# kupc25648/MOP-truss-MARL

Measured on AMD Instinct MI355X. Metric: env steps/sec (batched FEM solves) at 4096 envs, higher is better.
Workload: dtype f64; 1 GPU; synthetic random-geometry 2-row trusses, 32 nodes / 80 elements / 60 DOF, FEM-only env.step (action decode + FP64 assembly/solve + stresses + point), no agent; envs_per_gpu=4096, global_envs=4096, nodes=32, elements=80, ndof=60, half_bandwidth=7, lanes_per_env=16, rows_per_lane=1, parallelism=env-batch sharded over 1 GPU(s), no data-path collective

## Files before the change

mop-truss-marl_amd/csrc/truss_body.h:

```cpp
#pragma once
#include <stdint.h>
#include <math.h>

#ifndef TB_SCHED_FENCE
#define TB_SCHED_FENCE()
#endif
#ifndef TRUSS_HD
#error "define TRUSS_HD (e.g. __device__ __forceinline__) before including truss_body.h"
#endif

#define TF_TOP 1
#define TF_RESX 2
#define TF_RESY 4
#define TF_LOAD_BRIDGE 8
#define TF_LOAD_ROOF 16

#define TB_NO_DECODE 0x1u
#define TB_CLAMP_INPLACE 0x2u
#define TB_EMIT_OBS 0x4u

#if defined(__clang__)
typedef uint32_t tb_u4 __attribute__((ext_vector_type(4)));
typedef uint32_t tb_u2 __attribute__((ext_vector_type(2)));
typedef float tb_f4 __attribute__((ext_vector_type(4)));
// ... 512 lines not shown
      S[a] = m;
      S[b] = m;
    }
  }

  TRUSS_HD double load_at(const TopoDev &T, int r) const {
    if (r < 0 || r >= T.ndof) return 0.0;
    int nd = t_posnode(T)[r];
    if (nd < 0) return 0.0;
    int fl = t_nflags(T)[nd >> 1] & (is_roof ? TF_LOAD_ROOF : TF_LOAD_BRIDGE);
    if (!fl) return 0.0;
    return (nd & 1) ? load_y : load_x;
  }
  TRUSS_HD int orig_pos(const TopoDev &T, int tm, int p) const { return tm ? T.ndof - 1 - p : p; }
  TRUSS_HD double team_load(const TopoDev &T, int tm, int p) const {
    if (T.nteams == 1) return load_at(T, p);
    if (tm == 0) return p < T.ndof - T.KA ? load_at(T, p) : 0.0;
    return p < T.KA ? load_at(T, T.ndof - 1 - p) : 0.0;
  }

  static constexpr bool EBATCH = RPL == 1 && W <= 8 && EPL <= 5;
  static constexpr int ECH = EBATCH ? EPL : 1;
  TRUSS_HD void phase_elements(const TopoDev &T, const StepArgsDev &A) {
    const float *Y = ysh(T), *X = xsh(T);
    const int32_t *S = secsh(T);
    const int16_t *CN = t_conn(T);
    const double *AR = t_area(T), *ISR = t_isr(T);
    double *K = kb(T);
    const int16_t *AC = t_asm(T);
    double *EV = evsh(T);
    if (g == 0) EV[3 * T.E] = EV[3 * T.E + 1] = EV[3 * T.E + 2] = 0.0;
#pragma unroll
    for (int c0 = 0; c0 < EPL; c0 += ECH) {
      int n0[ECH], n1[ECH], sc[ECH], ev[ECH];
      tb_u2 code[ECH];
      float x0[ECH], x1[ECH], y0[ECH], y1[ECH];
      double Aa[ECH];
#pragma unroll
      for (int j = 0; j < ECH; ++j) {
        const int i = c0 + j < EPL ? c0 + j : EPL - 1;
        const int e = g + G * i;
        const int ee = e < T.E ? e : T.E - 1;
        const uint32_t c = *(const uint32_t *)(CN + 2 * ee);
        n0[j] = (int)(int16_t)(c & 0xffffu);
        n1[j] = (int)(int16_t)(c >> 16);
        sc[j] = S[ee];
        code[j] = *(const tb_u2 *)(AC + 4 * ee);
        ev[j] = 3 * ee;
      }
#pragma unroll
      for (int j = 0; j < ECH; ++j) {
        x0[j] = X[n0[j]];
        x1[j] = X[n1[j]];
        y0[j] = Y[n0[j]];
        y1[j] = Y[n1[j]];
        Aa[j] = AR[sc[j]];
      }
#pragma unroll
      for (int j = 0; j < ECH; ++j) {
        const int i = c0 + j;
        if (i < EPL) {
          const double dx = (double)x1[j] - (double)x0[j];
          const double dy = (double)y1[j] - (double)y0[j];
          const double l2 = dx * dx + dy * dy;
          const double rl = tb_rsqrt(l2);
          const double len = l2 * rl;
          const double c = dx * rl, s = dy * rl;
          const double k = (T.e_mod * Aa[j]) * rl;
          ek[i] = k;
          ec[i] = c;
          es[i] = s;
          ei[i] = ISR[sc[j]];
          if constexpr (EMIT) el[i] = (float)len;
          const double vol = (double)(float)(Aa[j] * len);
          if constexpr (EBATCH) p_vol += (g + G * i < T.E) ? vol : 0.0;
          else if (g + G * i < T.E) p_vol += vol;
          const double kc = k * c, ks = k * s;
          const double kcc = kc * c, kcs = kc * s, kss = ks * s;
          EV[ev[j] + 0] = kcc;
          EV[ev[j] + 1] = kcs;
          EV[ev[j] + 2] = kss;
          K[(int16_t)(code[j][0] & 0xffffu)] = -kcc;
          K[(int16_t)(code[j][0] >> 16)] = -kss;
          K[(int16_t)(code[j][1] & 0xffffu)] = -kcs;
          K[(int16_t)(code[j][1] >> 16)] = -kcs;
        }
      }
    }
  }

  TRUSS_HD void phase_assemble_nodes(const TopoDev &T) {
    const double *EV = evsh(T);
    const int16_t *AD = t_adj8(T), *DO = t_diagoff(T);
    double *K = kb(T);
    static_assert(NDEG == 8, "adjacency rows are read as one 16-byte unit");
    tb_u4 adj[NPL];
    int dof[NPL][3];
    double cc[NPL], cs[NPL], ss[NPL];
#pragma unroll
    for (int i = 0; i < NPL; ++i) {
      const int n0 = g + G * i, n = n0 < T.N ? n0 : T.N - 1;
      adj[i] = *(const tb_u4 *)(AD + n * NDEG);
      dof[i][0] = DO[3 * n];
      dof[i][1] = DO[3 * n + 1];
      dof[i][2] = DO[3 * n + 2];
      cc[i] = cs[i] = ss[i] = 0.0;
    }
#pragma unroll
    for (int h = 0; h < 2; ++h) {
      double ev[NPL][4][3];
#pragma unroll
      for (int i = 0; i < NPL; ++i)
#pragma unroll
        for (int a = 0; a < 4; ++a) {
          const uint32_t w = adj[i][2 * h + (a >> 1)];
          const int e = (a & 1) ? (int)(w >> 16) : (int)(w & 0xffffu);
          ev[i][a][0] = EV[3 * e + 0];
          ev[i][a][1] = EV[3 * e + 1];
          ev[i][a][2] = EV[3 * e + 2];
        }
#pragma unroll
      for (int i = 0; i < NPL; ++i)
#pragma unroll
        for (int a = 0; a < 4; ++a) {
          cc[i] += ev[i][a][0];
          cs[i] += ev[i][a][1];
          ss[i] += ev[i][a][2];
        }
    }
#pragma unroll
    for (int i = 0; i < NPL; ++i) {
      K[dof[i][0]] = cc[i];
      K[dof[i][1]] = ss[i];
      K[dof[i][2]] = cs[i];
    }
    for (int n = g + G * NPL; n < T.N; n += G) {
      double c2 = 0.0, s2 = 0.0, x2 = 0.0;
#pragma unroll
      for (int a = 0; a < NDEG; ++a) {
        const int e = AD[n * NDEG + a];
        c2 += EV[3 * e + 0];
        x2 += EV[3 * e + 1];
        s2 += EV[3 * e + 2];
      }
      K[DO[3 * n]] = c2;
      K[DO[3 * n + 1]] = s2;
      K[DO[3 * n + 2]] = x2;
    }
    const int idA = T.nteams == 1 ? T.ndof : T.ndof - T.KA;
    for (int r = idA + g; r < T.rowsA; r += G) K[r * W + r % W] = 1.0;
    for (int r = T.KA + T.mid + g; r < T.rowsB; r += G) K[(T.rowsA + r) * W + r % W] = 1.0;
  }

  TRUSS_HD void solver_scratch_init(const TopoDev &T) {
    double *Z = zs(T);
    const uint8_t *ZC = t_zcode(T);
    const int lbit = is_roof ? 4 : 2;
    {
      const int zt = T.zlen * T.nteams;
      constexpr int ZIT = 6;
#pragma unroll
      for (int i = 0; i < ZIT; ++i) {
        const int r0 = g + G * i, r = r0 < zt ? r0 : zt - 1;
        const int c = ZC[r];
        Z[r] = (c & lbit) ? ((c & 1) ? load_y : load_x) : 0.0;
      }
      for (int r = g + G * ZIT; r < zt; r += G) {
        const int c = ZC[r];
        Z[r] = (c & lbit) ? ((c & 1) ? load_y : load_x) : 0.0;
      }
    }
    tb_d2 *X2 = (tb_d2 *)__builtin_assume_aligned(xsol(T), 16);
    const tb_d2 z2 = {0.0, 0.0};
    for (int r = g; r < (T.zslot + 2) / 2; r += G) X2[r] = z2;
    double *RB = rbuf(T);
    for (int i = g; i < T.n_rest; i += G) RB[i] = 0.0;
  }

  TRUSS_HD void solver_init(const TopoDev &T) {
#pragma unroll
    for (int s = 0; s < RPL; ++s) {
      int r = gs + WL * s;
#pragma unroll
      for (int c = 0; c < W; ++c) R[s][c] = (c <= r) ? Kt[r * W + c] : Kt[c * W + r];
      rhs[s] = Zt[r];
    }
#pragma unroll
    for (int j = 0; j < W; ++j) xs[j] = 0.0;
  }

  double zkeep[RPL];
  TRUSS_HD void pivot_write(const TopoDev &T, int k, int kk) {
#pragma unroll
    for (int s = 0; s < RPL; ++s) Kt[k * W + gs + WL * s] = R[s][kk];
    bx = rhs[kk / WL];
  }
  TRUSS_HD void factor_z_store(const TopoDev &T, int kb, int c, int cnt) {
#pragma unroll
    for (int s = 0; s < RPL; ++s) {
      const int off = (gs + WL * s - c + W) % W;
      double *zp = off < cnt ? Zt + kb + off : ZRt + gs;
      *zp = zkeep[s];
    }
  }

  TRUSS_HD void pivot_update(const TopoDev &T, int k, int kk) {
    double col[W];
    {
      const double *Kn = Kt + (k + W) * W;
#pragma unroll
      for (int s = 0; s < RPL; ++s) ecol[s] = Kn[gs + WL * s];
    }
#pragma unroll
    for (int i = 0; i < W / 2; ++i) {
      tb_d2 v = ((const tb_d2 *)__builtin_assume_aligned(Kt + k * W, 16))[i];
      col[2 * i] = v[0];
      col[2 * i + 1] = v[1];
    }
    const double zk = tb_team_bcast(*this, kk % WL);
    if (gs == kk % WL) zkeep[kk / WL] = bx;
    const double d = col[kk];
    const double inv = tb_rcp(d);
#pragma unroll
    for (int s = 0; s < RPL; ++s) {
      double l = R[s][kk] * inv;
#pragma unroll
      for (int j = 0; j < W; ++j)
        if (j != kk) R[s][j] = fma(-l, col[j], R[s][j]);
      rhs[s] = fma(-l, zk, rhs[s]);
    }
#pragma unroll
    for (int s = 0; s < RPL; ++s) R[s][kk] = ecol[s];
    if (gs == kk % WL) {
      const int sp = kk / WL;
#pragma unroll
      for (int j = 0; j < W; ++j)
        if (j != kk) R[sp][j] = fr[sp][j];
      rhs[sp] = frhs[sp];
    }
  }
  double fr[RPL][W], frhs[RPL], ecol[RPL];
  TRUSS_HD void factor_rows_fetch(const TopoDev &T, int kb) {
#pragma unroll
    for (int s = 0; s < RPL; ++s) {
      const int rn = kb + W + gs + WL * s;
      const tb_d2 *K2 = (const tb_d2 *)__builtin_assume_aligned(Kt + rn * W, 16);
#pragma unroll
      for (int i = 0; i < W / 2; ++i) {
        tb_d2 v = K2[i];
        fr[s][2 * i] = v[0];
        fr[s][2 * i + 1] = v[1];
      }
      frhs[s] = Zt[rn];
    }
  }

  TRUSS_HD void pivot_check(const TopoDev &T) {
    const int lim = (T.nteams == 2 && team == 1) ? T.KA : (T.nteams == 2 ? T.KA + W : T.KA);
    for (int k = gs; k < lim; k += WL) {
      const double d = Kt[k * W + k % W];
      if (!(d > 0.0) || !(d < 1.7e308)) bad = 1;
    }
  }

  TRUSS_HD int win_row(const TopoDev &T, int slot) const { return T.KA + ((slot - T.KA % W + W) % W); }
  TRUSS_HD void merge_post(const TopoDev &T) {
    if (team == 1) {
      double *M = (double *)(L + T.o_mrg);
#pragma unroll
      for (int j = 0; j < W; ++j) M[gs * W + j] = R[0][j];
      M[W * W + gs] = rhs[0];
    }
  }
  TRUSS_HD void merge_take(const TopoDev &T) {
    if (team == 0) {
      const double *M = (const double *)(L + T.o_mrg);
      const int lim = T.ndof - T.KA;
      const int p = win_row(T, gs);
      const int pb = T.ndof - 1 - p;
#pragma unroll
      for (int j = 0; j < W; ++j) {
        const int c = win_row(T, j);
        const int cb = T.ndof - 1 - c;
        const bool ok = p < lim && c < lim;
        const double add = M[ok ? (pb % W) * W + (cb % W) : 0];
        R[0][j] += ok ? add : 0.0;
      }
      const double az = M[W * W + (p < lim ? pb % W : 0)];
      rhs[0] += p < lim ? az : 0.0;
    }
  }

  double bc[RPL][W], bz[RPL], bd[RPL];
  double nc[RPL][W], nz[RPL], nd[RPL];
  double bx;
  double myx[RPL] = {};
  TRUSS_HD void backsub_rows_fetch(const TopoDev &T, int kb) {
#pragma unroll
    for (int s = 0; s < RPL; ++s) {
      const int p = kb + gs + WL * s;
      const int pc = p < 0 ? 0 : p;
      const tb_d2 *K2 = (const tb_d2 *)__builtin_assume_aligned(Kt + pc * W, 16);
#pragma unroll
      for (int i = 0; i < W / 2; ++i) {
        tb_d2 v = K2[i];
        nc[s][2 * i] = v[0];
        nc[s][2 * i + 1] = v[1];
      }
      nz[s] = Zt[pc];
      nd[s] = Kt[pc * W + pc % W];
    }
  }
  TRUSS_HD void backsub_rows_adopt() {
#pragma unroll
    for (int s = 0; s < RPL; ++s) {
#pragma unroll
      for (int j = 0; j < W; ++j) bc[s][j] = nc[s][j];
      bz[s] = nz[s];
      bd[s] = tb_rcp(nd[s]);
    }
  }
  TRUSS_HD void backsub_step(const TopoDev &T, int k, int kk) {
    const int s = kk / WL;
    double acc0 = bz[s], acc1 = 0.0;
#pragma unroll
    for (int m = W - 1; m >= 2; --m) {
      const int j = (kk + m) % W;
      if (m & 1) acc1 = fma(-bc[s][j], xs[j], acc1);
      else acc0 = fma(-bc[s][j], xs[j], acc0);
    }
    const int jn = (kk + 1) % W;
    double acc = fma(-bc[s][jn], xs[jn], acc0 + acc1);
    bx = acc * bd[s];
  }
  TRUSS_HD void backsub_share(int kk) {
    xs[kk] = tb_team_bcast(*this, kk % WL);
    if (gs == kk % WL) myx[kk / WL] = bx;
  }
  TRUSS_HD bool owns_row(const TopoDev &T, int p) const {
    if (T.nteams == 1) return true;
    return team == 0 ? p < T.ndof - T.KA : p < T.KA;
  }
  TRUSS_HD void backsub_flush(const TopoDev &T, int kb) {
    double *XS = xsol(T);
#pragma unroll
    for (int s = 0; s < RPL; ++s) {
      const int p = kb + gs + WL * s;
      XS[owns_row(T, p) ? orig_pos(T, team, p) : T.zslot + 1] = myx[s];
    }
  }
  TRUSS_HD void backsub_flush_mid(const TopoDev &T) {
    double *XS = xsol(T);
    const int p = win_row(T, gs);
    XS[(team == 0 && owns_row(T, p)) ? p : T.zslot + 1] = myx[0];
  }
  TRUSS_HD void backsub_reload(const TopoDev &T) {
    const double *XS = xsol(T);
#pragma unroll
    for (int j = 0; j < W; ++j) {
      const int o = orig_pos(T, team, win_row(T, j));
      xs[j] = XS[(o >= 0 && o < T.ndof) ? o : T.zslot];
    }
  }

  TRUSS_HD float *oq0(const TopoDev &T) { return (float *)(L + T.o_kb + T.so_q0); }
  TRUSS_HD float *osr(const TopoDev &T) { return (float *)(L + T.o_kb + T.so_sr); }
  TRUSS_HD float *odisp(const TopoDev &T) { return (float *)(L + T.o_kb + T.so_disp); }
  TRUSS_HD float *omu(const TopoDev &T) { return (float *)(L + T.o_kb + T.so_mu); }
  TRUSS_HD float *omd(const TopoDev &T) { return (float *)(L + T.o_kb + T.so_md); }
  TRUSS_HD uint8_t *ocomp(const TopoDev &T) { return (uint8_t *)(L + T.o_kb + T.so_comp); }

  TRUSS_HD void phase_post_elements(const TopoDev &T, const StepArgsDev &A) {
    const double *XS = xsol(T);
    const int16_t *EX = t_exs(T);
    float *Q = oq0(T), *SR = osr(T);
    uint8_t *CP = ocomp(T);
    tb_u2 ex[EPL];
    double qv[EPL];
    float srv[EPL];
#pragma unroll
    for (int i = 0; i < EPL; ++i) {
      const int e = g + G * i;
      const int ee = e < T.E ? e : T.E - 1;
      ex[i] = *(const tb_u2 *)(EX + 4 * ee);
    }
    double v[EPL][4];
#pragma unroll
    for (int i = 0; i < EPL; ++i) {
      v[i][0] = XS[ex[i][0] & 0xffffu];
      v[i][1] = XS[ex[i][0] >> 16];
      v[i][2] = XS[ex[i][1] & 0xffffu];
      v[i][3] = XS[ex[i][1] >> 16];
    }
#pragma unroll
    for (int i = 0; i < EPL; ++i) {
      const double c = ec[i], s = es[i], k = ek[i];
      const double u0 = c * v[i][0] + s * v[i][1];
      const double u2 = c * v[i][2] + s * v[i][3];
      const double q = k * u0 + (-k) * u2;
      qv[i] = q;
      srv[i] = (float)(fabs(q) * ei[i]);
      p_c1 = fmaxf(p_c1, fabsf(srv[i]));
    }
#pragma unroll
    for (int i = 0; i < EPL; ++i) {
      const int e = g + G * i;
      const int ee = e < T.E ? e : T.E - 1;
      Q[ee] = (float)qv[i];
      SR[ee] = srv[i];
      CP[ee] = qv[i] > 0.0 ? 1 : 0;
      if constexpr (EMIT) {
        const bool cmp = qv[i] > 0.0;
        const float val = fminf(srv[i], 1.0f) * (srv[i] > 1.0f ? 1.0f : 0.5f);
        const tb_f2 tc = {cmp ? 0.0f : val, cmp ? val : 0.0f};
        ((tb_f2 *)((float *)L + T.b_tc))[ee] = tc;
        pe_sr[i] = srv[i];
        pe_cmp = i == 0 ? (cmp ? 1u : 0u) : (pe_cmp | (cmp ? 1u << i : 0u));
      }
    }
    if constexpr (EMIT) {
      if (g == 0) {
        const tb_f2 z = {0.0f, 0.0f};
        ((tb_f2 *)((float *)L + T.b_tc))[T.E] = z;
      }
    }
    if (A.q064 && active) {
      const size_t be = (size_t)envc * T.E;
#pragma unroll
      for (int i = 0; i < EPL; ++i) {
        const int e = g + G * i;
        if (e < T.E) A.q064[be + e] = qv[i];
      }
    }
    if (A.react) {
      const int16_t *CN = t_conn(T), *RS = t_restslot(T);
#pragma unroll
      for (int i = 0; i < EPL; ++i) {
        const int e = g + G * i;
        if (e < T.E) {
          const int n0 = CN[2 * e], n1 = CN[2 * e + 1];
          const double q = qv[i], c = ec[i], s = es[i];
          const int s0 = RS[2 * n0], s1 = RS[2 * n0 + 1];
          const int s2 = RS[2 * n1], s3 = RS[2 * n1 + 1];
          if (s0 >= 0) tb_lds_add(&rbuf(T)[s0], q * c);
          if (s1 >= 0) tb_lds_add(&rbuf(T)[s1], q * s);
          if (s2 >= 0) tb_lds_add(&rbuf(T)[s2], q * (-c));
          if (s3 >= 0) tb_lds_add(&rbuf(T)[s3], q * (-s));
        }
      }
    }
  }

  TRUSS_HD void phase_post_nodes(const TopoDev &T, const StepArgsDev &A) {
    const double *XS = xsol(T);
    const float *Y = ysh(T), *TG = tgsh(T);
    const int16_t *DP = t_dofpos(T), *PR = t_pairs(T);
    const uint8_t *NF = t_nflags(T);
    const size_t bn = (size_t)envc * T.N;
    const int zslot = T.zslot;
    float *DS = odisp(T), *MU = omu(T), *MD = omd(T);
    int px[NPL], py[NPL], fl[NPL];
    float yv[NPL], tg[NPL];
    double dxv[NPL], dyv[NPL];
#pragma unroll
    for (int i = 0; i < NPL; ++i) {
      const int n0 = g + G * i, n = n0 < T.N ? n0 : T.N - 1;
      px[i] = DP[2 * n];
      py[i] = DP[2 * n + 1];
      fl[i] = NF[n];
      yv[i] = Y[n];
      tg[i] = TG[n];
    }
#pragma unroll
    for (int i = 0; i < NPL; ++i) {
      dxv[i] = XS[px[i] < 0 ? zslot : px[i]];
      dyv[i] = XS[py[i] < 0 ? zslot : py[i]];
    }
#pragma unroll
    for (int i = 0; i < NPL; ++i) {
      const int n0 = g + G * i, n = n0 < T.N ? n0 : T.N - 1;
      const bool real = n0 < T.N, top = fl[i] & TF_TOP;
      const double dt = (double)fabsf(tg[i] - yv[i]);
      const float dr = fabsf((float)(dyv[i] / max_def));
      p_dt += (real && top) ? dt : 0.0;
      p_c2 = top ? p_c2 : fmaxf(p_c2, dr);
      DS[2 * n + 0] = (float)dxv[i];
      DS[2 * n + 1] = (float)dyv[i];
    }
    if (A.disp64 && active) {
#pragma unroll
      for (int i = 0; i < NPL; ++i) {
        const int n = g + G * i;
        if (n < T.N) {
          A.disp64[(bn + n) * 2 + 0] = dxv[i];
          A.disp64[(bn + n) * 2 + 1] = dyv[i];
        }
      }
    }
    for (int n = g + G * NPL; n < T.N; n += G) {
      const int qx = DP[2 * n], qy = DP[2 * n + 1];
      const double dx = XS[qx < 0 ? zslot : qx], dy = XS[qy < 0 ? zslot : qy];
      const float y = Y[n];
      if (NF[n] & TF_TOP) p_dt += (double)fabsf(TG[n] - y);
      else p_c2 = fmaxf(p_c2, fabsf((float)(dy / max_def)));
      DS[2 * n + 0] = (float)dx;
      DS[2 * n + 1] = (float)dy;
      if (A.disp64 && active) {
        A.disp64[(bn + n) * 2 + 0] = dx;
        A.disp64[(bn + n) * 2 + 1] = dy;
      }
    }
    if (A.mu_out && T.has_pairs) {
      constexpr int PPL = (NPL + 1) / 2;
#pragma unroll
// ... 270 lines not shown
        const int nc = n < T.N ? n : T.N - 1;
        const int fl = NFL[nc];
        const float y = Y[nc];
        float *f = nfe[i];
        f[0] = X[nc];
        f[1] = y;
        f[2] = (fl & lbit) ? 1.0f : 0.0f;
        f[3] = MU[nc];
        f[4] = MD[nc];
        f[5] = (fl & TF_TOP) ? TG[nc] / (y + 1e-6f) : 0.0f;
        f[6] = fabsf(DS[2 * nc + 1]);
        const float ratio = f[6] / maxdef32;
        f[7] = fminf(ratio, 1.0f) * (ratio > 1.0f ? 1.0f : 0.5f);
        f[8] = ratio > 1.0f ? 1.0f : 0.0f;
        const tb_f4 raw = {f[2], f[5], f[6], ratio >= 1.0f ? 1.0f : 0.0f};
        ((tb_f4 *)(Lf + T.b_nraw))[nc] = raw;
        if (n < T.N) {
#pragma unroll
          for (int c = 0; c < NDYN; ++c) {
            pmn[c] = fminf(pmn[c], f[c]);
            pmx[c] = fmaxf(pmx[c], f[c]);
          }
        }
      }
    }
  }

  TRUSS_HD void obs_bank_fill(const TopoDev &T, const StepArgsDev &A) {
    if constexpr (EMIT) {
      float *Lf = (float *)L;
      float nv[NPL][NDYN];
#pragma unroll
      for (int c = 0; c < NDYN; ++c) {
        const float lo = tb_group_min(*this, c), hi = tb_group_max(*this, c);
        const float inv = tb_rcpf(hi - lo + 1e-6f);
#pragma unroll
        for (int i = 0; i < NPL; ++i) nv[i][c] = (nfe[i][c] - lo) * inv;
      }
#pragma unroll
      for (int i = 0; i < NPL; ++i) {
        const int n = g + G * i;
        const int nc = n < T.N ? n : T.N - 1;
        const tb_f4 a = {nv[i][0], nv[i][1], nv[i][2], nv[i][3]}, b = {nv[i][4], nv[i][5], nv[i][6], nv[i][7]};
        ((tb_f4 *)(Lf + T.b_nna))[nc] = a;
        ((tb_f4 *)(Lf + T.b_nnb))[nc] = b;
        Lf[T.b_nn8 + nc] = nv[i][8];
      }
    }
  }

  TRUSS_HD tb_f4 gather4(const float *Lf, const tb_u2 t) const {
    const tb_f4 v = {Lf[t[0] & 0xffffu], Lf[t[0] >> 16], Lf[t[1] & 0xffffu], Lf[t[1] >> 16]};
    return v;
  }
  template <int IT>
  TRUSS_HD void emit_rows(float *out, size_t row_floats, int nc, const tb_u2 (&tab)[IT]) const {
    if (!out) return;
    const float *Lf = (const float *)L;
    tb_f4 *o4 = (tb_f4 *)(out + (size_t)env * row_floats);
#pragma unroll
    for (int b0 = 0; b0 < IT; b0 += KB) {
      if (b0 * G < nc) {
        tb_f4 v[KB];
#pragma unroll
        for (int k = 0; k < KB; ++k)
          if (b0 + k < IT) v[k] = gather4(Lf, tab[b0 + k]);
#pragma unroll
        for (int k = 0; k < KB; ++k)
          if (b0 + k < IT) TB_OBS_STORE(&o4[chunk_of(b0 + k, nc)], v[k]);
      }
    }
  }
  TRUSS_HD void obs_nxe_table(const TopoDev &T) {
    if constexpr (EMIT) {
      if (T.nxe_cw != 4) return;
      const tb_u2 *tab = TB_TAB(tb_u2, TB, T.f_tnxe);
#pragma unroll
      for (int i = 0; i < IE; ++i) ete[i] = tab[i * G + g];
    }
  }
  TRUSS_HD void emit_nxe_narrow(const TopoDev &T, const StepArgsDev &A) const {
    if (!A.nxe) return;
    const float *Lf = (const float *)L;
    const uint16_t *tab = TB_TAB(uint16_t, TB, T.f_tnxe);
    float *o = A.nxe + (size_t)env * 21 * T.E;
    const int nc = T.nc_nxe;
    if (T.nxe_cw == 2) {
      for (int q0 = g; q0 < nc; q0 += 4 * G) {
        tb_f2 v[4];
#pragma unroll
        for (int k = 0; k < 4; ++k) {
          const int q = q0 + k * G < nc ? q0 + k * G : nc - 1;
          const tb_f2 w = {Lf[tab[2 * q]], Lf[tab[2 * q + 1]]};
          v[k] = w;
        }
#pragma unroll
        for (int k = 0; k < 4; ++k) {
          const int q = q0 + k * G < nc ? q0 + k * G : nc - 1;
          TB_OBS_STORE((tb_f2 *)o + q, v[k]);
        }
      }
    } else {
      for (int q0 = g; q0 < nc; q0 += 4 * G) {
        float v[4];
#pragma unroll
        for (int k = 0; k < 4; ++k) v[k] = Lf[tab[q0 + k * G < nc ? q0 + k * G : nc - 1]];
#pragma unroll
        for (int k = 0; k < 4; ++k) TB_OBS_STORE(o + (q0 + k * G < nc ? q0 + k * G : nc - 1), v[k]);
      }
    }
  }
  TRUSS_HD void obs_emit_raw_rows(const TopoDev &T, const StepArgsDev &A) {
    if constexpr (EMIT) {
      if (!active) return;
      if (T.nxe_cw == 4) emit_rows<IE>(A.nxe, (size_t)21 * T.E, T.nc_nxe, ete);
      else emit_nxe_narrow(T, A);
      emit_rows<IN_>(A.nxn, (size_t)12 * T.N, T.nc_nxn, etn);
    }
  }
  TRUSS_HD void obs_emit_xn(const TopoDev &T, const StepArgsDev &A) {
    if constexpr (EMIT) {
      if (!active) return;
      emit_rows<IX>(A.x_n, (size_t)13 * T.N, T.nc_xn, etx);
    }
  }
};

#ifndef TRUSS_ST
#define TRUSS_ST(i)
#endif
#define TRUSS_STREAM_SEG1(PH, T, A) PH(obs_emit_as(T, A));
#define TRUSS_STREAM_SEG2(PH, T, A) \
  PH(obs_emit_tc(T, A));            \
  PH(obs_nxe_table(T));
#define TRUSS_STREAM_SEG3(PH, T, A) \
  PH(obs_emit_raw_rows(T, A));      \
  PH(obs_emit_xn(T, A));
#define TRUSS_STEP_SCHEDULE(PH, PH_NS, BAR, T, A)                                   \
  TRUSS_ST(0);                                                                      \
  PH(phase_stage(T, A));                                                            \
  TRUSS_ST(1);                                                                      \
  PH(phase_decode(T, A));                                                           \
  if ((T).n_sym_nodes > 0 && !((A).flags & TB_NO_DECODE)) { PH(phase_sym_nodes(T)); } \
  TRUSS_ST(2);                                                                      \
  PH(phase_sizing(T, A));                                                           \
  if ((T).n_sym_elems > 0 && !((A).flags & TB_NO_DECODE)) { PH(phase_sym_elems(T)); } \
  if (EMIT_) { EMIT_POINT(1); TRUSS_ST(19); }  \
  PH_NS(rollout_prefetch(T, A));  \
  TRUSS_ST(3);                                                                      \
  PH(phase_elements(T, A));                                                         \
  TRUSS_ST(10);                                                                     \
  PH(phase_assemble_nodes(T));                                                      \
  TRUSS_ST(11);                                                                     \
  PH(solver_scratch_init(T));                                                       \
  TRUSS_ST(4);                                                                      \
  PH(solver_init(T));                                                               \
  {                                                                                 \
                                                                                    \
    const int kend_ = (T).nteams == 2 ? (T).KA + W_ : (T).KA;                       \
    int kb_ = 0;                                                                    \
    for (; kb_ + W_ <= (T).KA; kb_ += W_) {                                         \
      PH_NS(factor_rows_fetch(T, kb_));                                             \
      TRUSS_UNROLL                                                                  \
      for (int kk_ = 0; kk_ < W_; ++kk_) {                                          \
        PH(pivot_write(T, kb_ + kk_, kk_));                                         \
        PH_NS(pivot_update(T, kb_ + kk_, kk_));                                     \
      }                                                                             \
      PH_NS(factor_z_store(T, kb_, 0, W_));                                         \
    }                                                                               \
    TRUSS_ST(13);                                                                   \
                                  \
    if ((T).nteams == 2 && W_ <= 8) {                                               \
      const int c0_ = (T).KA % W_;                                                  \
      TRUSS_UNROLL                                                                  \
      for (int c_ = 0; c_ < W_; ++c_) {                                             \
        if (c_ == c0_) {                                                            \
          if (c_ > 0) { PH_NS(factor_rows_fetch(T, kb_)); }                         \
          TRUSS_UNROLL                                                              \
          for (int kk_ = 0; kk_ < c_; ++kk_) {                                      \
            PH(pivot_write(T, kb_ + kk_, kk_));                                     \
            PH_NS(pivot_update(T, kb_ + kk_, kk_));                                 \
          }                                                                         \
          if (c_ > 0) { PH_NS(factor_z_store(T, kb_, 0, c_)); }                     \
          PH(merge_post(T));                                                        \
          PH(merge_take(T));                                                        \
          TRUSS_UNROLL                                                              \
          for (int i_ = 0; i_ < W_; ++i_) {                                         \
            if ((c_ + i_) % W_ == 0) { PH_NS(factor_rows_fetch(T, (T).KA + i_)); }  \
            PH(pivot_write(T, (T).KA + i_, (c_ + i_) % W_));                        \
            PH_NS(pivot_update(T, (T).KA + i_, (c_ + i_) % W_));                    \
          }                                                                         \
          PH_NS(factor_z_store(T, (T).KA, c_, W_));                                 \
        }                                                                           \
      }                                                                             \
    } else if ((T).nteams == 2) {  \
      for (; kb_ < kend_; kb_ += W_) {                                              \
        PH_NS(factor_rows_fetch(T, kb_));                                           \
        TRUSS_UNROLL                                                                \
        for (int kk_ = 0; kk_ < W_; ++kk_) {                                        \
          if (kb_ + kk_ < kend_) {                                                  \
            if (kb_ + kk_ == (T).KA) {                                              \
              PH(merge_post(T));                                                    \
              PH(merge_take(T));                                                    \
            }                                                                       \
            PH(pivot_write(T, kb_ + kk_, kk_));                                     \
            PH_NS(pivot_update(T, kb_ + kk_, kk_));                                 \
          }                                                                         \
        }                                                                           \
        PH_NS(factor_z_store(T, kb_, 0, kend_ - kb_ < W_ ? kend_ - kb_ : W_));      \
      }                                                                             \
    }                                                                               \
    BAR();                                                                          \
    PH_NS(pivot_check(T));                                                          \
    TRUSS_ST(5);                                                                    \
                \
    kb_ = ((kend_ - 1) / W_) * W_;                                                  \
    PH_NS(backsub_rows_fetch(T, kb_));                                              \
    if ((T).nteams == 2 && W_ <= 8) {                                               \
      const int c0_ = (T).KA % W_;                                                  \
      TRUSS_UNROLL                                                                  \
      for (int c_ = 0; c_ < W_; ++c_) {                                             \
        if (c_ == c0_) {                                                            \
          PH_NS(backsub_rows_adopt());                                              \
          PH_NS(backsub_rows_fetch(T, kb_ - W_));                                   \
          TRUSS_UNROLL                                                              \
          for (int i_ = W_ - 1; i_ >= 0; --i_) {                                    \
            PH_NS(backsub_step(T, (T).KA + i_, (c_ + i_) % W_));                    \
            PH_NS(backsub_share((c_ + i_) % W_));                                   \
            if ((c_ + i_) % W_ == 0 && i_ > 0) {         \
              kb_ -= W_;                                                            \
              PH_NS(backsub_rows_adopt());                                          \
              PH_NS(backsub_rows_fetch(T, kb_ - W_));                               \
            }                                                                       \
          }                                                                         \
          PH_NS(backsub_flush_mid(T));                                              \
          BAR();                                                                    \
          PH_NS(backsub_reload(T));                                                 \
          TRUSS_UNROLL                                                              \
          for (int kk_ = c_ - 1; kk_ >= 0; --kk_) {                                 \
            PH_NS(backsub_step(T, kb_ + kk_, kk_));                                 \
            PH_NS(backsub_share(kk_));                                              \
          }                                                                         \
          if (c_ > 0) { PH_NS(backsub_flush(T, kb_)); }                             \
          kb_ -= W_;                                                                \
        }                                                                           \
      }                                                                             \
    } else if ((T).nteams == 2) {                                                   \
      for (; kb_ >= 0 && kb_ + W_ - 1 >= (T).KA - 1; kb_ -= W_) {                   \
        PH_NS(backsub_rows_adopt());                                                \
        PH_NS(backsub_rows_fetch(T, kb_ - W_));                                     \
        TRUSS_UNROLL                                                                \
        for (int kk_ = W_ - 1; kk_ >= 0; --kk_) {                                   \
          if (kb_ + kk_ < kend_) {                                                  \
            if (kb_ + kk_ == (T).KA - 1) {                                          \
              PH_NS(backsub_flush_mid(T));                                          \
              BAR();                                                                \
              PH_NS(backsub_reload(T));                                             \
            }                                                                       \
            PH_NS(backsub_step(T, kb_ + kk_, kk_));                                 \
            PH_NS(backsub_share(kk_));                                              \
          }                                                                         \
        }                                                                           \
        PH_NS(backsub_flush(T, kb_));                                               \
      }                                                                             \
    }                                                                               \
    TRUSS_ST(14);                                                                   \
    for (; kb_ >= 0; kb_ -= W_) {                                                   \
      PH_NS(backsub_rows_adopt());                                                  \
      PH_NS(backsub_rows_fetch(T, kb_ - W_));                                       \
      TRUSS_UNROLL                                                                  \
      for (int kk_ = W_ - 1; kk_ >= 0; --kk_) {                                     \
        PH_NS(backsub_step(T, kb_ + kk_, kk_));                                     \
        PH_NS(backsub_share(kk_));                                                  \
      }                                                                             \
      PH_NS(backsub_flush(T, kb_));                                                 \
    }                                                                               \
  }                                                                                 \
  BAR();                                                                            \
  TRUSS_ST(6);                                                                      \
  PH_NS(rollout_stash(T, A));                                                       \
  PH(phase_post_elements(T, A));                                                    \
  if (EMIT_) {                                                                      \
    EMIT_POINT(2);                                                                  \
    TRUSS_ST(18);                                                                   \
    PH(obs_elements_bank(T, A));                                                    \
  }                                                                                 \
  TRUSS_ST(7);                                                                      \
  PH(phase_post_nodes(T, A));                                                       \
  TRUSS_ST(8);                                                                      \
  if (EMIT_) {   \
    TRUSS_ST(15);                                                                   \
    PH(obs_nodes_raw(T, A));                                                        \
    TRUSS_ST(16);                                                                   \
    PH(obs_bank_fill(T, A));                                                        \
    EMIT_POINT(3);                                                                  \
    TRUSS_ST(17);                                                                   \
  }                                                                                 \
  PH_NS(phase_finish(T, A));                                                        \
  TRUSS_ST(12);                                                                     \
  PH_NS(phase_store(T, A));                                                         \
  TRUSS_ST(9);

struct ObsArgsDev {
  int32_t B;
  uint32_t flags;
  const float *x, *y;
  const int32_t *sec;
  const float *mu, *md, *target, *disp, *q0, *sr;
  const uint8_t *comp;
  const double *env_params;
  float *x_n, *A_s, *A_ts, *A_cs, *nxn, *nxe;
  int32_t tile_rows;
  int32_t n_split;
};

struct ObsLane {
  int lane, env;
  char *L;
  float maxdef32;
  int is_roof;
  int role;
  int minmax_done;

  TRUSS_HD float *raw() { return (float *)L; }
  TRUSS_HD float *mn(const TopoDev &T) { return raw() + T.N * 13; }
  TRUSS_HD float *mx(const TopoDev &T) { return mn(T) + 13; }
  TRUSS_HD float *part(const TopoDev &T) { return mx(T) + 13; }
  TRUSS_HD float *mats(const TopoDev &T) { return (float *)(L + (((size_t)(T.N * 13 + 26 + 128) * 4 + 15) & ~(size_t)15)); }

  TRUSS_HD void init(int lane_, int block, int tile, const TopoDev &, const ObsArgsDev &A, char *lds) {
    lane = lane_;
    env = block;
    L = lds;
    role = A.n_split <= 1 ? 0 : tile == 0 ? 2 : 1;
    minmax_done = 0;
    const double *P = A.env_params + (size_t)env * 8;
    maxdef32 = (float)P[2];
    is_roof = P[7] != 0.0;
  }

  TRUSS_HD void phase_nodes(const TopoDev &T, const ObsArgsDev &A) {
    if (role == 1) return;
    const size_t bn = (size_t)env * T.N;
    float *R = raw();
    for (int n = lane; n < T.N; n += 64) {
      const int fl = TB_TAB(uint8_t, T.blob, T.f_nflags)[n];
      const float top = (fl & TF_TOP) ? 1.0f : 0.0f;
      const float y = A.y[bn + n];
      float f[13];
      f[0] = A.x[bn + n];
      f[1] = y;
      f[2] = (fl & TF_RESX) ? 1.0f : 0.0f;
      f[3] = (fl & TF_RESY) ? 1.0f : 0.0f;
      f[4] = (fl & (is_roof ? TF_LOAD_ROOF : TF_LOAD_BRIDGE)) ? 1.0f : 0.0f;
      f[5] = top;
      f[6] = 1.0f - top;
      f[7] = A.mu[bn + n];
      f[8] = A.md[bn + n];
      f[9] = (fl & TF_TOP) ? A.target[bn + n] / (y + 1e-6f) : 0.0f;
      f[10] = fabsf(A.disp[(bn + n) * 2 + 1]);
      const float ratio = f[10] / maxdef32;
      f[11] = fminf(ratio, 1.0f) * (ratio > 1.0f ? 1.0f : 0.5f);
      f[12] = ratio > 1.0f ? 1.0f : 0.0f;
#pragma unroll
      for (int c = 0; c < 13; ++c) R[n * 13 + c] = f[c];
      if (A.nxn) {
        float *o = A.nxn + (bn + n) * 12;
#pragma unroll
        for (int c = 0; c < 11; ++c) o[c] = f[c];
        o[11] = ratio >= 1.0f ? 1.0f : 0.0f;
      }
    }
  }

  TRUSS_HD void phase_tile_clear(const TopoDev &T, const ObsArgsDev &A) {
    if (role != 1 && !minmax_done) {
      const int c = lane & 15, q = lane >> 4;
      if (c < 13) {
        const float *R = raw();
        float lo = R[c], hi = R[c];
        for (int n = q; n < T.N; n += 4) {
          const float v = R[n * 13 + c];
          lo = fminf(lo, v);
          hi = fmaxf(hi, v);
        }
        part(T)[q * 16 + c] = lo;
        part(T)[64 + q * 16 + c] = hi;
      }
    }
    if (role == 2) return;
    float *M = mats(T);
    const int tot = 3 * A.tile_rows * T.N;
    if ((tot & 3) == 0) {
      tb_u4 *M4 = (tb_u4 *)M;
      const tb_u4 z = {0u, 0u, 0u, 0u};
      for (int i = lane; i < tot / 4; i += 64) M4[i] = z;
    } else {
      for (int i = lane; i < tot; i += 64) M[i] = 0.0f;
    }
  }

  TRUSS_HD void phase_edges(const TopoDev &T, const ObsArgsDev &A, int r0) {
    const float *R = raw();
    const int TR = A.tile_rows;
    if (r0 == 0 && role != 1) {
      if (lane < 13) {
        const float *P = part(T);
        mn(T)[lane] = fminf(fminf(P[lane], P[16 + lane]), fminf(P[32 + lane], P[48 + lane]));
        mx(T)[lane] = fmaxf(fmaxf(P[64 + lane], P[80 + lane]), fmaxf(P[96 + lane], P[112 + lane]));
      }
      minmax_done = 1;
    }
    const size_t be = (size_t)env * T.E;
    float *As = mats(T), *Ats = As + TR * T.N, *Acs = Ats + TR * T.N;
    const double *AR = TB_TAB(double, T.blob, T.f_area);
    const int16_t *CN = TB_TAB(int16_t, T.blob, T.f_conn);
    const double amax = AR[T.n_sections - 1];
    if (role == 1) {
      const int16_t *ADJ = TB_TAB(int16_t, T.blob, T.f_adj8);
      for (int i = lane; i < TR * 8; i += 64) {
        const int n = r0 + (i >> 3);
// ... 104 lines not shown
```

mop-truss-marl_amd/csrc/truss_hip.hip:

```cpp
#include <hip/hip_runtime.h>

#include <atomic>
#include <cstdint>
#include <cstdio>
#include <cstring>
#include <type_traits>

#include "../../include/truss_mi355.h"

#pragma clang fp contract(off)

#define TRUSS_HD __device__ __forceinline__
#define TRUSS_UNROLL _Pragma("unroll")
#define TB_SCHED_FENCE() __builtin_amdgcn_sched_barrier(0)
#define TB_STREAM_STORE(p, v) __builtin_nontemporal_store((v), (p))
#ifdef TRUSS_OBS_STORE_NT
#define TB_OBS_STORE(p, v) __builtin_nontemporal_store((v), (p))
#else
#define TB_OBS_STORE(p, v) (*(p) = (v))
#endif

__device__ __forceinline__ void tb_lds_add(double *p, double v) { unsafeAtomicAdd(p, v); }

template <int WL, int SRC>
__device__ __forceinline__ double tb_dpp_bcast(double v) {
  const int lo = __double2loint(v), hi = __double2hiint(v);
  int rlo, rhi;
  if constexpr (WL == 16) {
    rlo = __builtin_amdgcn_update_dpp(lo, lo, 0x150 + SRC, 0xf, 0xf, false);
    rhi = __builtin_amdgcn_update_dpp(hi, hi, 0x150 + SRC, 0xf, 0xf, false);
  } else if constexpr (WL == 8) {
    rlo = __builtin_amdgcn_update_dpp(lo, lo, 0x150 + SRC, 0xf, 0x3, false);
    rlo = __builtin_amdgcn_update_dpp(rlo, lo, 0x150 + 8 + SRC, 0xf, 0xc, false);
    rhi = __builtin_amdgcn_update_dpp(hi, hi, 0x150 + SRC, 0xf, 0x3, false);
    rhi = __builtin_amdgcn_update_dpp(rhi, hi, 0x150 + 8 + SRC, 0xf, 0xc, false);
  } else {
    static_assert(WL == 4, "team width");
    constexpr int qp = SRC | (SRC << 2) | (SRC << 4) | (SRC << 6);
    rlo = __builtin_amdgcn_update_dpp(lo, lo, qp, 0xf, 0xf, false);
    rhi = __builtin_amdgcn_update_dpp(hi, hi, qp, 0xf, 0xf, false);
  }
  return __hiloint2double(rhi, rlo);
}
template <class LN>
__device__ __forceinline__ double tb_team_bcast(LN &ln, int src) {
  constexpr int WL = LN::WL_;
  switch (src) {
#define TB_CASE(i) \
  case i:          \
    if constexpr (i < WL) return tb_dpp_bcast<WL, i>(ln.bx); else break;
    TB_CASE(0) TB_CASE(1) TB_CASE(2) TB_CASE(3) TB_CASE(4) TB_CASE(5) TB_CASE(6) TB_CASE(7)
    TB_CASE(8) TB_CASE(9) TB_CASE(10) TB_CASE(11) TB_CASE(12) TB_CASE(13) TB_CASE(14) TB_CASE(15)
#undef TB_CASE
  }
  return ln.bx;
}

__device__ __forceinline__ double tb_rcp(double d) {
  double r = __builtin_amdgcn_rcp(d);
  r = fma(fma(-d, r, 1.0), r, r);
  r = fma(fma(-d, r, 1.0), r, r);
  return r;
}

__device__ __forceinline__ float tb_rcpf(float d) {
  float r = __builtin_amdgcn_rcpf(d);
  return fmaf(fmaf(-d, r, 1.0f), r, r);
}

#ifdef TRUSS_STOP_AT
#define TRUSS_ST(i) do { if ((i) == TRUSS_STOP_AT) return; } while (0)
#endif
#ifdef TRUSS_STAMPS
__device__ unsigned long long g_truss_stamps[32];
__device__ unsigned long long g_truss_span[4096][6];
#define TRUSS_ST(i)                                                  \
  do {                                                               \
    __builtin_amdgcn_sched_barrier(0);                               \
    if (threadIdx.x == 0 && blockIdx.x == gridDim.x / 2) g_truss_stamps[i] = clock64(); \
    if (threadIdx.x == 0 && ((i) == 0 || (i) == 9) && blockIdx.x < 4096) {              \
      g_truss_span[blockIdx.x][(i) == 0 ? 0 : 2] = clock64();                            \
      g_truss_span[blockIdx.x][(i) == 0 ? 1 : 3] = wall_clock64();                       \
    }                                                                \
    __builtin_amdgcn_sched_barrier(0);                               \
  } while (0)
#endif

__device__ __forceinline__ double tb_rsqrt(double x) {
  double r = __builtin_amdgcn_rsq(x);
  r = r * fma(-0.5 * x, r * r, 1.5);
  r = r * fma(-0.5 * x, r * r, 1.5);
  return r;
}

template <int G, bool MAX>
__device__ __forceinline__ float tb_group_reduce(float v) {
  auto op = [](float a, float b) { return MAX ? fmaxf(a, b) : fminf(a, b); };
  auto dpp = [](float x, auto ctrl) {
    return __int_as_float(__builtin_amdgcn_update_dpp(0, __float_as_int(x), decltype(ctrl)::value, 0xf, 0xf, false));
  };
  if constexpr (G >= 2) v = op(v, dpp(v, std::integral_constant<int, 0xB1>{}));
  if constexpr (G >= 4) v = op(v, dpp(v, std::integral_constant<int, 0x4E>{}));
  if constexpr (G >= 8) v = op(v, dpp(v, std::integral_constant<int, 0x141>{}));
  if constexpr (G >= 16) v = op(v, dpp(v, std::integral_constant<int, 0x140>{}));
  if constexpr (G >= 32) v = op(v, __shfl_xor(v, 16));
  if constexpr (G >= 64) v = op(v, __shfl_xor(v, 32));
  return v;
}
template <class LN>
__device__ __forceinline__ float tb_group_min(LN &ln, int c) { return tb_group_reduce<LN::G_, false>(ln.pmn[c]); }
template <class LN>
__device__ __forceinline__ float tb_group_max(LN &ln, int c) { return tb_group_reduce<LN::G_, true>(ln.pmx[c]); }

template <int G>
__device__ __forceinline__ double tb_group_reduce_sum(double v) {
  auto dpp = [](double x, auto ctrl) {
    const int lo = __builtin_amdgcn_update_dpp(0, __double2loint(x), decltype(ctrl)::value, 0xf, 0xf, false);
    const int hi = __builtin_amdgcn_update_dpp(0, __double2hiint(x), decltype(ctrl)::value, 0xf, 0xf, false);
    return __hiloint2double(hi, lo);
  };
  if constexpr (G >= 2) v = v + dpp(v, std::integral_constant<int, 0xB1>{});
  if constexpr (G >= 4) v = v + dpp(v, std::integral_constant<int, 0x4E>{});
  if constexpr (G >= 8) v = v + dpp(v, std::integral_constant<int, 0x141>{});
  if constexpr (G >= 16) v = v + dpp(v, std::integral_constant<int, 0x140>{});
  if constexpr (G >= 32) v = v + __shfl_xor(v, 16);
  if constexpr (G >= 64) v = v + __shfl_xor(v, 32);
  return v;
}
template <class LN>
__device__ __forceinline__ double tb_group_sum_d(LN &ln, int which) {
  return tb_group_reduce_sum<LN::G_>(which == 0 ? ln.p_vol : which == 1 ? ln.p_dt : ln.p_en);
}
template <class LN>
__device__ __forceinline__ float tb_group_max_f(LN &ln, int which) {
  return tb_group_reduce<LN::G_, true>(which == 0 ? ln.p_c1 : which == 1 ? ln.p_c2 : (float)ln.bad);
}

template <class LN, class TD>
__device__ __forceinline__ bool tb_obs_timed_out(LN &ln, const TD &T) {
  if constexpr (LN::EMIT_) return *((const __attribute__((address_space(3))) int *)(ln.TB + T.o_flag) + 1) != 0;
  return false;
}

#include "truss_body.h"

typedef __attribute__((address_space(3))) int tb_lds_word;
__device__ __forceinline__ tb_lds_word *tb_flag_ptr(char *lds, int o_flag) { return (tb_lds_word *)(lds + o_flag); }
__device__ __forceinline__ void tb_publish(char *lds, int o_flag, int k) {
  __builtin_amdgcn_wave_barrier();
#ifdef TRUSS_FLAG_RELAXED
  __builtin_amdgcn_fence(__ATOMIC_RELEASE, "wavefront");
  if (threadIdx.x == 0) __hip_atomic_store(tb_flag_ptr(lds, o_flag), k, __ATOMIC_RELAXED, __HIP_MEMORY_SCOPE_WORKGROUP);
#else
  if (threadIdx.x == 0) __hip_atomic_store(tb_flag_ptr(lds, o_flag), k, __ATOMIC_RELEASE, __HIP_MEMORY_SCOPE_WORKGROUP);
#endif
}
#ifndef TB_AWAIT_SPINS
#define TB_AWAIT_SPINS (1 << 22)
#endif
__device__ __forceinline__ bool tb_await(char *lds, int o_flag, int k) {
  for (int spin = 0; spin < TB_AWAIT_SPINS; ++spin) {
    const int v = __hip_atomic_load(tb_flag_ptr(lds, o_flag), __ATOMIC_ACQUIRE, __HIP_MEMORY_SCOPE_WORKGROUP);
    if (__builtin_amdgcn_readfirstlane(v) >= k) return true;
    __builtin_amdgcn_s_sleep(1);
  }
  return false;
}

template <class LN>
__device__ __forceinline__ void tb_obs_timeout(LN &ln, char *lds, int o_flag, int32_t *status) {
  if ((threadIdx.x & 63) == 0) *(tb_flag_ptr(lds, o_flag) + 1) = 1;
  if (ln.g == 0 && ln.active && status) atomicOr(&status[ln.env], TRUSS_STATUS_OBS_TIMEOUT);
}

#define TB_WAVE_SYNC()                                    \
  do {                                                    \
    __builtin_amdgcn_fence(__ATOMIC_RELEASE, "wavefront"); \
    __builtin_amdgcn_wave_barrier();                      \
    __builtin_amdgcn_fence(__ATOMIC_ACQUIRE, "wavefront"); \
  } while (0)
#define PH(call) \
  ln.call;       \
  TB_WAVE_SYNC()
#define PH_NS(call) ln.call
#define BAR() TB_WAVE_SYNC()

template <int G, int WL, int RPL, int EPL, bool EMIT>
__global__ __launch_bounds__(EMIT ? 128 : 64) void truss_step_kernel(const TopoDev T, const StepArgsDev A) {
  extern __shared__ __attribute__((aligned(16))) char smem[];
  StepLane<G, WL, RPL, EPL, EMIT> ln;
  ln.init(threadIdx.x & 63, blockIdx.x, T, A, smem);
  constexpr int W_ = StepLane<G, WL, RPL, EPL, EMIT>::W;
  constexpr bool EMIT_ = EMIT;
  if constexpr (EMIT) {
    if (threadIdx.x == 0) {
// ... 227 lines not shown
```

Before: 232.5 million env-steps/s.

## Compute load RHS on the fly, fold pivot check into backsub, use 64-bit DPP

Removes the scratch pass that materialised the load vector Z and zeroed the solution buffer. The RHS is now generated from the zcode table when rows are fetched, with a prefetch of the next code. The separate pivot-check pass and its barrier are dropped, and the diagonal-positivity test moves into backsub_rows_adopt, where the diagonal is already loaded. Reaction-buffer zeroing now runs only when reactions are requested, and the 16- and 8-lane broadcasts use 64-bit DPP intrinsics instead of two 32-bit moves. The risk is correctness: the reload now reads only the middle solution range plus a zeroed slot, so any stale xsol entries it touches could feed wrong values.

```diff
diff --git a/mop-truss-marl_amd/csrc/truss_body.h b/mop-truss-marl_amd/csrc/truss_body.h
--- a/mop-truss-marl_amd/csrc/truss_body.h
+++ b/mop-truss-marl_amd/csrc/truss_body.h
@@ -688,30 +688,22 @@
     for (int r = T.KA + T.mid + g; r < T.rowsB; r += G) K[(T.rowsA + r) * W + r % W] = 1.0;
   }
 
-  TRUSS_HD void solver_scratch_init(const TopoDev &T) {
-    double *Z = zs(T);
-    const uint8_t *ZC = t_zcode(T);
+  TRUSS_HD void solver_scratch_init(const TopoDev &T, const StepArgsDev &A) {
+    xsol(T)[T.zslot] = 0.0;
+    if (A.react) {
+      double *RB = rbuf(T);
+      for (int i = g; i < T.n_rest; i += G) RB[i] = 0.0;
+    }
+  }
+  TRUSS_HD int z_code(const TopoDev &T, int r) const {
+    const int zt = T.zlen * T.nteams;
+    return t_zcode(T)[r < zt ? r : zt - 1];
+  }
+  TRUSS_HD double z_value(int c) const {
     const int lbit = is_roof ? 4 : 2;
-    {
-      const int zt = T.zlen * T.nteams;
-      constexpr int ZIT = 6;
-#pragma unroll
-      for (int i = 0; i < ZIT; ++i) {
-        const int r0 = g + G * i, r = r0 < zt ? r0 : zt - 1;
-        const int c = ZC[r];
-        Z[r] = (c & lbit) ? ((c & 1) ? load_y : load_x) : 0.0;
-      }
-      for (int r = g + G * ZIT; r < zt; r += G) {
-        const int c = ZC[r];
-        Z[r] = (c & lbit) ? ((c & 1) ? load_y : load_x) : 0.0;
-      }
-    }
-    tb_d2 *X2 = (tb_d2 *)__builtin_assume_aligned(xsol(T), 16);
-    const tb_d2 z2 = {0.0, 0.0};
-    for (int r = g; r < (T.zslot + 2) / 2; r += G) X2[r] = z2;
-    double *RB = rbuf(T);
-    for (int i = g; i < T.n_rest; i += G) RB[i] = 0.0;
-  }
+    return (c & lbit) ? ((c & 1) ? load_y : load_x) : 0.0;
+  }
+  TRUSS_HD double z_initial(const TopoDev &T, int r) const { return z_value(z_code(T, r)); }
 
   TRUSS_HD void solver_init(const TopoDev &T) {
 #pragma unroll
@@ -719,7 +711,8 @@
       int r = gs + WL * s;
 #pragma unroll
       for (int c = 0; c < W; ++c) R[s][c] = (c <= r) ? Kt[r * W + c] : Kt[c * W + r];
-      rhs[s] = Zt[r];
+      rhs[s] = z_initial(T, team * T.zlen + r);
+      if constexpr (ZAHEAD) fcode[s] = z_code(T, team * T.zlen + W + r);
     }
 #pragma unroll
     for (int j = 0; j < W; ++j) xs[j] = 0.0;
@@ -775,7 +768,9 @@
       rhs[sp] = frhs[sp];
     }
   }
+  static constexpr bool ZAHEAD = !EMIT;
   double fr[RPL][W], frhs[RPL], ecol[RPL];
+  int fcode[RPL];
   TRUSS_HD void factor_rows_fetch(const TopoDev &T, int kb) {
 #pragma unroll
     for (int s = 0; s < RPL; ++s) {
@@ -787,15 +782,12 @@
         fr[s][2 * i] = v[0];
         fr[s][2 * i + 1] = v[1];
       }
-      frhs[s] = Zt[rn];
-    }
-  }
-
-  TRUSS_HD void pivot_check(const TopoDev &T) {
-    const int lim = (T.nteams == 2 && team == 1) ? T.KA : (T.nteams == 2 ? T.KA + W : T.KA);
-    for (int k = gs; k < lim; k += WL) {
-      const double d = Kt[k * W + k % W];
-      if (!(d > 0.0) || !(d < 1.7e308)) bad = 1;
+      if constexpr (ZAHEAD) {
+        frhs[s] = z_value(fcode[s]);
+        fcode[s] = z_code(T, team * T.zlen + rn + W);
+      } else {
+        frhs[s] = z_initial(T, team * T.zlen + rn);
+      }
     }
   }
 
@@ -847,13 +839,16 @@
       nd[s] = Kt[pc * W + pc % W];
     }
   }
-  TRUSS_HD void backsub_rows_adopt() {
+  TRUSS_HD void backsub_rows_adopt(const TopoDev &T, int kb) {
+    const int lim = (T.nteams == 2 && team == 1) ? T.KA : (T.nteams == 2 ? T.KA + W : T.KA);
 #pragma unroll
     for (int s = 0; s < RPL; ++s) {
 #pragma unroll
       for (int j = 0; j < W; ++j) bc[s][j] = nc[s][j];
       bz[s] = nz[s];
       bd[s] = tb_rcp(nd[s]);
+      const bool notpos = !(nd[s] > 0.0) || !(nd[s] < 1.7e308);
+      bad |= (kb + gs + WL * s < lim && notpos) ? 1 : 0;
     }
   }
   TRUSS_HD void backsub_step(const TopoDev &T, int k, int kk) {
@@ -895,7 +890,7 @@
 #pragma unroll
     for (int j = 0; j < W; ++j) {
       const int o = orig_pos(T, team, win_row(T, j));
-      xs[j] = XS[(o >= 0 && o < T.ndof) ? o : T.zslot];
+      xs[j] = XS[(o >= T.KA && o < T.ndof - T.KA) ? o : T.zslot];
     }
   }
 
@@ -1472,7 +1467,7 @@
   TRUSS_ST(10);                                                                     \
   PH(phase_assemble_nodes(T));                                                      \
   TRUSS_ST(11);                                                                     \
-  PH(solver_scratch_init(T));                                                       \
+  PH(solver_scratch_init(T, A));                                                    \
   TRUSS_ST(4);                                                                      \
   PH(solver_init(T));                                                               \
   {                                                                                 \
@@ -1530,8 +1525,6 @@
         PH_NS(factor_z_store(T, kb_, 0, kend_ - kb_ < W_ ? kend_ - kb_ : W_));      \
       }                                                                             \
     }                                                                               \
-    BAR();                                                                          \
-    PH_NS(pivot_check(T));                                                          \
     TRUSS_ST(5);                                                                    \
                 \
     kb_ = ((kend_ - 1) / W_) * W_;                                                  \
@@ -1541,7 +1534,7 @@
       TRUSS_UNROLL                                                                  \
       for (int c_ = 0; c_ < W_; ++c_) {                                             \
         if (c_ == c0_) {                                                            \
-          PH_NS(backsub_rows_adopt());                                              \
+          PH_NS(backsub_rows_adopt(T, kb_));                                              \
           PH_NS(backsub_rows_fetch(T, kb_ - W_));                                   \
           TRUSS_UNROLL                                                              \
           for (int i_ = W_ - 1; i_ >= 0; --i_) {                                    \
@@ -1549,7 +1542,7 @@
             PH_NS(backsub_share((c_ + i_) % W_));                                   \
             if ((c_ + i_) % W_ == 0 && i_ > 0) {         \
               kb_ -= W_;                                                            \
-              PH_NS(backsub_rows_adopt());                                          \
+              PH_NS(backsub_rows_adopt(T, kb_));                                          \
               PH_NS(backsub_rows_fetch(T, kb_ - W_));                               \
             }                                                                       \
           }                                                                         \
@@ -1567,7 +1560,7 @@
       }                                                                             \
     } else if ((T).nteams == 2) {                                                   \
       for (; kb_ >= 0 && kb_ + W_ - 1 >= (T).KA - 1; kb_ -= W_) {                   \
-        PH_NS(backsub_rows_adopt());                                                \
+        PH_NS(backsub_rows_adopt(T, kb_));                                                \
         PH_NS(backsub_rows_fetch(T, kb_ - W_));                                     \
         TRUSS_UNROLL                                                                \
         for (int kk_ = W_ - 1; kk_ >= 0; --kk_) {                                   \
@@ -1586,7 +1579,7 @@
     }                                                                               \
     TRUSS_ST(14);                                                                   \
     for (; kb_ >= 0; kb_ -= W_) {                                                   \
-      PH_NS(backsub_rows_adopt());                                                  \
+      PH_NS(backsub_rows_adopt(T, kb_));                                                  \
       PH_NS(backsub_rows_fetch(T, kb_ - W_));                                       \
       TRUSS_UNROLL                                                                  \
       for (int kk_ = W_ - 1; kk_ >= 0; --kk_) {                                     \
diff --git a/mop-truss-marl_amd/csrc/truss_hip.hip b/mop-truss-marl_amd/csrc/truss_hip.hip
--- a/mop-truss-marl_amd/csrc/truss_hip.hip
+++ b/mop-truss-marl_amd/csrc/truss_hip.hip
@@ -24,23 +24,22 @@
 
 template <int WL, int SRC>
 __device__ __forceinline__ double tb_dpp_bcast(double v) {
-  const int lo = __double2loint(v), hi = __double2hiint(v);
-  int rlo, rhi;
   if constexpr (WL == 16) {
-    rlo = __builtin_amdgcn_update_dpp(lo, lo, 0x150 + SRC, 0xf, 0xf, false);
-    rhi = __builtin_amdgcn_update_dpp(hi, hi, 0x150 + SRC, 0xf, 0xf, false);
+    const long long x = __double_as_longlong(v);
+    return __longlong_as_double(__builtin_amdgcn_update_dpp(x, x, 0x150 + SRC, 0xf, 0xf, false));
   } else if constexpr (WL == 8) {
-    rlo = __builtin_amdgcn_update_dpp(lo, lo, 0x150 + SRC, 0xf, 0x3, false);
-    rlo = __builtin_amdgcn_update_dpp(rlo, lo, 0x150 + 8 + SRC, 0xf, 0xc, false);
-    rhi = __builtin_amdgcn_update_dpp(hi, hi, 0x150 + SRC, 0xf, 0x3, false);
-    rhi = __builtin_amdgcn_update_dpp(rhi, hi, 0x150 + 8 + SRC, 0xf, 0xc, false);
+    const long long x = __double_as_longlong(v);
+    long long r = __builtin_amdgcn_update_dpp(x, x, 0x150 + SRC, 0xf, 0x3, false);
+    r = __builtin_amdgcn_update_dpp(r, x, 0x150 + 8 + SRC, 0xf, 0xc, false);
+    return __longlong_as_double(r);
   } else {
     static_assert(WL == 4, "team width");
+    const int lo = __double2loint(v), hi = __double2hiint(v);
     constexpr int qp = SRC | (SRC << 2) | (SRC << 4) | (SRC << 6);
-    rlo = __builtin_amdgcn_update_dpp(lo, lo, qp, 0xf, 0xf, false);
-    rhi = __builtin_amdgcn_update_dpp(hi, hi, qp, 0xf, 0xf, false);
-  }
-  return __hiloint2double(rhi, rlo);
+    const int rlo = __builtin_amdgcn_update_dpp(lo, lo, qp, 0xf, 0xf, false);
+    const int rhi = __builtin_amdgcn_update_dpp(hi, hi, qp, 0xf, 0xf, false);
+    return __hiloint2double(rhi, rlo);
+  }
 }
 template <class LN>
 __device__ __forceinline__ double tb_team_bcast(LN &ln, int src) {
```

Measured after the change: 232.1 million env-steps/s. No clear change (-0.1%).
